# subhk/FeastKit.jl

Measured on AMD Instinct MI355X. Metric: eigenpairs/sec + max residual, 16-node contour, higher is better.
Workload: dtype f64

## Files before the change

feastkit.jl_amd/_lib.py:

```python
from __future__ import annotations

import ctypes as C
import os

_HERE = os.path.dirname(os.path.abspath(__file__))
LIB_PATH = os.environ.get("FEASTHIP_LIB") or os.path.join(_HERE, "libfeasthip.so")


class FeastHipStats(C.Structure):
    _fields_ = [
        ("seconds_total", C.c_double),
        ("seconds_solve", C.c_double),
        ("krylov_iterations", C.c_int64),
        ("spmm_calls", C.c_int64),
        ("factorizations", C.c_int64),
        ("max_rel_residual", C.c_double),
    ]

    def asdict(self):
        return {k: getattr(self, k) for k, _ in self._fields_}


class FeastHipPolicy(C.Structure):
    _fields_ = [("Emin", C.c_double), ("Emax", C.c_double), ("inner_rtol", C.c_double), ("outer_tol", C.c_double),
# ... 46 lines not shown
    "feasthip_project_dev": (_i, [_vp, _i64, _vp, _i, _i, _vp, _vp]),
    "feasthip_ritz_residual": (_i, [_vp, _i64, _vp, _vp, _vp, _i64, _i, _i, _vp, _vp]),
    "feasthip_ritz_residual_dev": (_i, [_vp, _i64, _vp, _vp, _vp, _i64, _i, _i, _vp, _vp]),
    "feasthip_matmul": (_i, [_vp, _i, _i64, _vp, _vp]),
    "feasthip_matmul_dev": (_i, [_vp, _i, _i64, _vp, _vp]),
    "feasthip_band_plan": (_i, [_vp, _vp, _vp, _vp, _vp]),
    "feasthip_direct_plan_flops": (_i, [_vp, _vp]),
    "feasthip_release_factors": (_i, [_vp]),
    "feasthip_shifted_solve": (_i, [_vp, _d, _d, _i64, _vp, _vp, _ps]),
    "feasthip_shifted_solve_dev": (_i, [_vp, _d, _d, _i64, _vp, _vp, _ps]),
    "feasthip_last_node_iterations": (_i, [_vp, _vp, _i]),
    "feasthip_last_column_iterations": (_i, [_vp, _vp, _i]),
    "feasthip_last_global_node_iterations": (_i, [_vp, _vp, _i]),
    "feasthip_last_shifted_sweep": (_i, [_vp, _vp, _vp, _vp, _vp]),
    "feasthip_last_block_sweep": (_i, [_vp, _vp, _vp, _vp, _vp]),
    "feasthip_profile_enable": (_i, [_vp, _i]),
    "feasthip_profile_reset": (_i, [_vp]),
    "feasthip_profile_get": (_i, [_vp, C.c_char_p, _pd, _pi64]),
    "feasthip_profile_set_period": (_i, [_vp, _i]),
    "feasthip_profile_get_work": (_i, [_vp, C.c_char_p, _pd]),
    "feasthip_policy_init": (_i, [_vp, _d, _d, _i, _i, _d, _d, _i, _i, _i]),
    "feasthip_policy_update": (_i, [_vp, _d, _i, _i, _vp, _i]),
    "feasthip_policy_set_aside": (_i, [_vp, _i, _vp]),
    "feasthip_policy_pick_direct_nodes": (_i, [_vp, _i, _i, _d, _d, _d, _i, _vp]),
    "feasthip_policy_filter_ratio": (_d, [_d, _d, _i, _i, _i, _d, _vp, _i]),
    "feasthip_policy_reach": (_d, [_vp, _i, _d, _d, _d]),
}

UNIQUE_ID_BYTES = 128

# ... 29 lines not shown
```

feastkit.jl_amd/csrc/fh_api.hip:

```cpp
#include "fh_common.hpp"
#include "fh_kernels.hpp"
#include "fh_dense.hpp"
#include "fh_banded.hpp"
#include "fh_eig.hpp"
#include "fh_comm.hpp"
#include "fh_cholqr.hpp"
#include "fh_knobs.hpp"
#include "../../include/feasthip.h"

#include <algorithm>
#include <chrono>
#include <thread>
#include <cmath>
#include <cstring>

int fh_get_buf(feasthip_ctx* h, const char* name, size_t bytes, void** out) {
    auto it = h->bufs.find(name);
    if (it != h->bufs.end() && it->second.second >= bytes) {
        *out = it->second.first;
        return 0;
    }
    if (it != h->bufs.end()) {
        hipStreamSynchronize(h->stream);
        hipFree(it->second.first);
// ... 434 lines not shown


struct fh_op_call {
    const void* X = nullptr; size_t x_stride = 0;
    void* Y = nullptr; size_t y_stride = 0;
    const cplx* coefA = nullptr; const cplx* coefB = nullptr;
    const void* Bvec = nullptr; size_t b_stride = 0;
    const void* U = nullptr; size_t u_stride = 0;
    int dot_mode = 0; cplx* partial1 = nullptr; cplx* partial2 = nullptr;
    const int* node_active = nullptr;
    int nodes = 1;
    int m = FH_MAX_LD;
    int uniform_coef = 0;
    int prec = 64;
    const cplx* colscale = nullptr;
};

static bool fh_row_kernel_ok(feasthip_ctx* h, int ld) {
    return h->kind == 2 && ld == 64 && !h->csr.is_complex && h->csr.rp8 && fh_knob::spmm_row();
}

static int fh_apply_operator(feasthip_ctx* h, int ld, const fh_op_call& c) {
    if (h->kind == 2) {
        fh_spmm_args a;
        a.rowptr = h->csr.rowptr; a.col = h->csr.col; a.aval = h->csr.aval; a.bval = h->csr.bval;
        a.N = (int)h->csr.N; a.nodes = c.nodes;
        a.X = c.X; a.x_node_stride = c.x_stride; a.Y = c.Y; a.y_node_stride = c.y_stride;
        a.coefA = c.coefA; a.coefB = c.coefB; a.Bvec = c.Bvec; a.b_node_stride = c.b_stride;
        a.U = c.U; a.u_node_stride = c.u_stride; a.dot_mode = c.dot_mode;
        a.partial1 = c.partial1; a.partial2 = c.partial2; a.node_active = c.node_active;
        a.counters = h->profiling ? h->d_counters : nullptr; a.m = c.m; a.uniform_coef = c.uniform_coef; a.prec = c.prec;
        const bool lds_kernel = h->csr.lcol && c.prec == 64 && fh_knob::lds_spmm() && c.nodes <= 64 && c.dot_mode != 6;
        a.nblk_rows = h->csr.nblk; a.blk_start = h->csr.blk_start; a.ext_ptr = h->csr.ext_ptr; a.ext_idx = h->csr.ext_idx;
        a.lcol = lds_kernel ? h->csr.lcol : nullptr;
        a.use_row_kernel = (fh_row_kernel_ok(h, ld) && !lds_kernel) ? 1 : 0;
        a.colscale = c.colscale;
        if (c.colscale && (lds_kernel || c.prec != 64 || h->csr.is_complex)) { h->last_error = "internal: column-scaled operand needs a gather kernel over a real matrix on complex128 panels"; return -1; }
        a.rp8 = h->csr.rp8; a.col8 = h->csr.col8; a.a8 = h->csr.a8; a.b8 = h->csr.b8;
        fh_prof_begin(h, "spmm");
        fh_launch_spmm(a, ld, h->csr.is_complex != 0, h->csr.b_identity != 0, fh_spmm_grid(a.N, ld), h->stream);
        fh_prof_end(h);
        if (a.use_row_kernel) return fh_spmm_row_grid(a.N);
        if (lds_kernel) return (8 / (ld / 16)) * fh_spmm_lds_slots(a.nblk_rows, ld);
        return fh_spmm_partials(a.N, ld);
    }
    fh_dense_op_args a;
    a.A = h->dense.A; a.B = h->dense.B; a.N = (int)h->dense.N; a.is_complex = h->dense.is_complex;
    a.nodes = c.nodes; a.X = (const cplx*)c.X; a.x_node_stride = c.x_stride; a.Y = (cplx*)c.Y; a.y_node_stride = c.y_stride;
    a.coefA = c.coefA; a.coefB = c.coefB; a.Bvec = (const cplx*)c.Bvec; a.b_node_stride = c.b_stride;
    a.U = (const cplx*)c.U; a.u_node_stride = c.u_stride; a.dot_mode = c.dot_mode;
    a.partial1 = c.partial1; a.partial2 = c.partial2; a.node_active = c.node_active;
    int nblk = fh_dense_op_nblk(a.N);
    fh_prof_begin(h, "dense_op");
    fh_launch_dense_op(a, ld, nblk, h->stream);
    fh_prof_end(h);
    return nblk;
}

static int fh_op_nblk(feasthip_ctx* h, int ld) {
    if (h->kind == 2) return std::max(std::max(fh_spmm_partials((int)h->csr.N, ld), ld == 64 ? fh_spmm_row_grid((int)h->csr.N) : 0),
                                      h->csr.lcol ? (8 / (ld / 16)) * fh_spmm_lds_slots(h->csr.nblk, ld) : 0);
    return fh_dense_op_nblk((int)h->dense.N);
}
static const int* fh_perm(feasthip_ctx* h) { return h->kind == 2 ? h->csr.perm : nullptr; }
static int64_t fh_N(feasthip_ctx* h) { return h->kind == 2 ? h->csr.N : h->dense.N; }
static bool fh_b_identity(feasthip_ctx* h) { return h->kind == 2 ? h->csr.b_identity != 0 : h->dense.b_identity != 0; }

static int fh_check_problem(feasthip_ctx* h, int64_t m, int wide = 0) {
    if (!h) return FEASTHIP_ERROR_INTERNAL;
    if (h->poisoned) { h->last_error = "handle poisoned by an earlier device failure: destroy it"; return FEASTHIP_ERROR_INTERNAL; }
    if (h->kind == 0) { h->last_error = "no matrix set (feasthip_set_dense / feasthip_set_csr)"; return FEASTHIP_ERROR_N; }
    if (m <= 0 || (!wide && m > FH_MAX_LD) || m > fh_N(h)) {
        h->last_error = wide ? "block width m must satisfy 1 <= m <= N" : "block width m must satisfy 1 <= m <= min(N, 64)";
        return FEASTHIP_ERROR_M0;
    }
// ... 182 lines not shown
}

struct fh_krylov_opts {
    cplx* sum_acc = nullptr;
    const std::vector<cplx>* wnode = nullptr;
    const cplx *shared_src = nullptr, *dznode = nullptr;
    const double *shared_lambda = nullptr, *shared_lambda_host = nullptr;
};

namespace {
struct fh_krylov_work {
    feasthip_ctx* h;
    fh_solve_result& res;
    int method, prec, ld, m, nodes, N;
    size_t panel;
    bool fused = false, lazy = false;
    void *R, *Rh, *P, *V, *S, *T, *D = nullptr, *RHS32 = nullptr, *Xk = nullptr;
    fh_krylov_scalars s;
    double *r0_64, *inv_r0;
    cplx *part1, *part2, *sp[2] = {nullptr, nullptr};
    int nblk_vec, fv_rows = 0, fv1_rows = 0;
    cplx *sum_acc = nullptr, *dfs = nullptr;
    const cplx* lazy_src = nullptr;
    fh_op_call oc;
    fh_fin_args fa;
    fh_vec_args va;
    fh_fused_fin_args ff;
    int alloc(const std::vector<cplx>& z, const std::vector<cplx>* wnode);
    int start(const std::vector<cplx>& z, const cplx* RHS, cplx* X, const fh_krylov_opts& opt);
    void bicgstab_step(), cocg_step(), cocg_fused_step(int it);
};
// ... 73 lines not shown
        fh_launch_narrow_scaled((const cplx*)R64, panel, (cplxf*)RHS32, panel, r0_64, N, ld, nblk_vec, nodes, h->stream);
        FH_CHECK(hipMemsetAsync(D, 0, (size_t)nodes * panel * sizeof(cplxf), h->stream));
        FH_CHECK(hipMemcpyAsync(R, RHS32, (size_t)nodes * panel * sizeof(cplxf), hipMemcpyDeviceToDevice, h->stream));
        Xk = D;
        std::vector<double> hr0(nl), hinv(nl);
        FH_CHECK(hipMemcpyAsync(hr0.data(), r0_64, nl * sizeof(double), hipMemcpyDeviceToHost, h->stream));
        FH_CHECK(hipStreamSynchronize(h->stream));
        for (size_t i = 0; i < nl; ++i) hinv[i] = hr0[i] > 0 ? 1.0 / hr0[i] : 0.0;
        FH_CHECK(hipMemcpyAsync(inv_r0, hinv.data(), nl * sizeof(double), hipMemcpyHostToDevice, h->stream));
        FH_CHECK(hipStreamSynchronize(h->stream));
        fa.atol_scale = inv_r0;
    }
    va.X = Xk;
    lazy = shared_start && fused && h->kind == 2 && !h->csr.is_complex && !fh_knob::no_lazy_start() &&
           (!opt.shared_lambda || opt.shared_lambda_host) && !fh_knob::lds_spmm();
    if (lazy) {
        if ((rc = fh_upload_coefs(h, "kry_fscale", fh_start_factors(z, nodes, m, ld, opt.shared_lambda_host), &dfs))) return rc;
        lazy_src = opt.shared_src;
        fh_vec_args vs = va;
        vs.Q = opt.shared_src; vs.first_scale = dfs;
        fh_launch_cocg_init_lazy(vs, ld, nblk_vec, nodes, h->stream);
    } else if (shared_start) {
        fh_vec_args vs = va;
        vs.Q = opt.shared_src; vs.lambda = opt.shared_lambda; vs.znode = opt.dznode;
        fh_launch_cocg_init_shared(vs, ld, nblk_vec, nodes, h->stream);
    } else if (method == 1 || prec == 32) {
        fh_launch_cocg_init(va, ld, nblk_vec, nodes, h->stream);
    }
    if (method == 1 || prec == 32) fa.nblk = nblk_vec;
    fh_launch_fin_init(fa, ld, nodes, h->stream);
// ... 20 lines not shown
void fh_krylov_work::cocg_step() {
    oc.X = P; oc.Y = V; oc.U = nullptr; oc.dot_mode = 4; oc.node_active = s.node_active;
    fa.nblk = fh_apply_operator(h, ld, oc);
    fh_prof_begin(h, "dot_finalize"); fh_launch_fin_alpha(fa, ld, nodes, h->stream); fh_prof_end(h);
    fh_prof_begin(h, "cocg_xr"); fh_launch_cocg_update(va, ld, nblk_vec, nodes, h->stream); fh_prof_end(h);
    fa.nblk = nblk_vec;
    fh_prof_begin(h, "dot_finalize"); fh_launch_fin_rho(fa, ld, nodes, h->stream); fh_prof_end(h);
    fh_prof_begin(h, "cocg_p");
    if (sum_acc) fh_launch_cocg_p_sum(va, ld, nodes, h->stream);
    else fh_launch_cocg_p(va, ld, nblk_vec, nodes, h->stream);
    fh_prof_end(h);
    res.op_calls += 1;
}

void fh_krylov_work::cocg_fused_step(int it) {
    const bool first_lazy = lazy && it == 0;
    oc.X = first_lazy ? (const void*)lazy_src : P; oc.x_stride = first_lazy ? 0 : panel; oc.colscale = first_lazy ? dfs : nullptr;
    oc.Y = V; oc.U = nullptr; oc.dot_mode = 6; oc.node_active = s.node_active;
    oc.partial1 = sp[0]; oc.partial2 = sp[1];
    va.first_src = first_lazy ? lazy_src : nullptr; va.first_scale = first_lazy ? dfs : nullptr;
    ff.sig = sp[0]; ff.kap = sp[1]; ff.final_check = 0;
    ff.predict_stop = (h->rtol >= 1e-3 && h->atol == 0.0) ? 1 : 0;
    ff.nblk_op = fh_apply_operator(h, ld, oc);
    ff.nblk_vec = it == 0 ? fa.nblk : ((lazy && it == 1) ? fv1_rows : fv_rows);
    fh_prof_begin(h, "dot_finalize"); fh_launch_fused_fin(ff, ld, nodes, h->stream); fh_prof_end(h);
    fh_prof_begin(h, "cocg_vec"); fh_launch_fused_vec(va, ld, h->stream); fh_prof_end(h);
    res.op_calls += 1;
}

}

static int fh_krylov(feasthip_ctx* h, int method, int prec, int ld, int m, int nodes, const std::vector<cplx>& z,
                     const cplx* RHS, cplx* X, size_t stride, fh_solve_result& res, const fh_krylov_opts& opt) {
    if (h->kind != 2) prec = 64;
    fh_krylov_work k{h, res};
// ... 736 lines not shown
        if (dzAq) FH_CHECK(hipMemcpy(dzAq, aq_all.data(), aq_all.size() * sizeof(cplx), hipMemcpyHostToDevice));
        if (dzSq) FH_CHECK(hipMemcpy(dzSq, sq_all.data(), sq_all.size() * sizeof(cplx), hipMemcpyHostToDevice));
    }
    return 0;
}

struct fh_resident_sweep {
    const cplx* Q; const cplx* eigres; cplx* P; int ld;
};

static int fh_contour_apply_impl(feasthip_ctx* h, int64_t m64, const cplx* dQ, const double* ritz_lambda,
                                 cplx* dQproj, cplx* dzAq, cplx* dzSq, int* node_status, feasthip_stats* stats,
                                 const fh_resident_sweep* rs = nullptr) {
    h->shift_panels = h->shift_used = h->shift_seed_iters = 0; h->shift_seed = -1;
    h->block_panels = h->block_used = h->block_steps_max = h->block_breakdowns = h->block_passes = 0;
    const int nr = fh_comm_nranks(h);
    int64_t c0 = 0, c1 = m64;
    if (h->col_block_hi >= 0) { c0 = std::min(h->col_block_lo, m64); c1 = std::min(std::max(h->col_block_hi, c0), m64); }
    const bool full = (c0 == 0 && c1 == m64);
    if (nr == 1 && full) {
        if (rs) {
            fh_panel_io io; io.Qp = rs->Q; io.eigres = rs->eigres; io.out = rs->P;
            return fh_contour_apply_panel(h, m64, nullptr, ritz_lambda, nullptr, nullptr, nullptr, node_status, stats, nullptr, &io);
        }
        return fh_contour_apply_local(h, m64, dQ, ritz_lambda, dQproj, dzAq, dzSq, node_status, stats);
    }
    int rc = fh_check_problem(h, m64, rs ? 0 : 1);
    if (rc) return rc;
    if (!full && (dzAq || dzSq)) { h->last_error = "contour_apply: moment matrices need the full column block"; return FEASTHIP_ERROR_M0; }
    const int N = (int)fh_N(h), m = (int)m64, nodes = h->node_count, ne = (int)h->zne.size();
// ... 1370 lines not shown
    if (seed_iterations) *seed_iterations = u ? h->shift_seed_iters : 0;
    if (spmm_node_passes) *spmm_node_passes = u ? h->shift_seed_iters : 0;
    return 0;
}

extern "C" int feasthip_last_block_sweep(feasthip_handle h, int* used, int* node_steps_max, int* breakdown_nodes, int* spmm_node_passes) {
    if (!h) return FEASTHIP_ERROR_INTERNAL;
    const bool u = h->block_panels > 0 && h->block_used == h->block_panels;
    if (used) *used = u ? 1 : 0;
    if (node_steps_max) *node_steps_max = u ? h->block_steps_max : 0;
    if (breakdown_nodes) *breakdown_nodes = u ? h->block_breakdowns : 0;
    if (spmm_node_passes) *spmm_node_passes = u ? h->block_passes : 0;
    return 0;
}

extern "C" int feasthip_last_column_iterations(feasthip_handle h, int* out, int n) {
    if (!h || !out) return FEASTHIP_ERROR_INTERNAL;
    for (int e = 0; e < n; ++e) out[e] = e < (int)h->last_col_iters.size() ? h->last_col_iters[e] : 0;
    return 0;
}

extern "C" int feasthip_profile_enable(feasthip_handle h, int enable) {
    if (!h) return FEASTHIP_ERROR_INTERNAL;
    h->profiling = enable ? 1 : 0;
    if (enable) { h->prof_host_s = 0.0; h->prof_t0 = fh_now_s(); }
    return 0;
}
extern "C" int feasthip_profile_reset(feasthip_handle h) {
    if (!h) return FEASTHIP_ERROR_INTERNAL;
    fh_prof_collect(h);
// ... 41 lines not shown
```

feastkit.jl_amd/csrc/fh_common.hpp:

```cpp
#pragma once
#include <hip/hip_runtime.h>
#include <stdint.h>
#include <string>
#include <vector>
#include <map>

struct __attribute__((aligned(16))) cplx { double x, y; };

__host__ __device__ inline cplx cmake(double a, double b) { cplx r; r.x = a; r.y = b; return r; }
__host__ __device__ inline cplx cadd(cplx a, cplx b) { return cmake(a.x + b.x, a.y + b.y); }
__host__ __device__ inline cplx csub(cplx a, cplx b) { return cmake(a.x - b.x, a.y - b.y); }
__host__ __device__ inline cplx cmul(cplx a, cplx b) { return cmake(a.x * b.x - a.y * b.y, a.x * b.y + a.y * b.x); }
__host__ __device__ inline cplx cmulc(cplx a, cplx b) {  return cmake(a.x * b.x + a.y * b.y, a.x * b.y - a.y * b.x); }
__host__ __device__ inline cplx cscale(cplx a, double s) { return cmake(a.x * s, a.y * s); }
__host__ __device__ inline cplx cconj(cplx a) { return cmake(a.x, -a.y); }
__host__ __device__ inline double cabs2(cplx a) { return a.x * a.x + a.y * a.y; }
__host__ __device__ inline cplx cdiv(cplx a, cplx b) {
    double d = b.x * b.x + b.y * b.y;
    return cmake((a.x * b.x + a.y * b.y) / d, (a.y * b.x - a.x * b.y) / d);
}
__host__ __device__ inline void cfma(cplx& acc, cplx a, cplx b) {
    acc.x += a.x * b.x - a.y * b.y;
    acc.y += a.x * b.y + a.y * b.x;
}
// ... 95 lines not shown
    fh_csr csr;
    fh_dense dense;

    std::vector<cplx> zne, wne;
    double weight_scale = 2.0;
    int real_projection = 0;
    int node_first = 0, node_count = 0;
    std::vector<int> node_ids;
    std::vector<int> node_kinds;

    int solver = 1;
    int shifted = 0;
    int shift_panels = 0, shift_used = 0, shift_seed = -1, shift_seed_iters = 0;
    int block = 0;
    int block_panels = 0, block_used = 0, block_steps_max = 0, block_breakdowns = 0, block_passes = 0;
    double rtol = 1e-12, atol = 0.0;
    int maxit = 500, restart = 30, factor_precision = 64, cache_factors = 1;

    std::vector<int> last_col_iters;
    int last_col_m = 0;
    std::vector<int> last_node_iters;
    std::vector<int> global_node_iters;

    std::map<std::string, std::pair<void*, size_t>> bufs;

    char* pin = nullptr; size_t pin_cap = 0, pin_off = 0;

    int rs_m = 0, rs_ld = 0;
    cplx* rs_P = nullptr;
    cplx* rs_basis = nullptr;
// ... 65 lines not shown
```

feastkit.jl_amd/csrc/fh_kernels.hpp:

```cpp
#pragma once
#include "fh_common.hpp"

struct fh_spmm_args {
    const int* rowptr; const int* col; const void* aval; const void* bval;
    int N; int nodes;
    const void* X; size_t x_node_stride;
    void* Y; size_t y_node_stride;
    const cplx* coefA; const cplx* coefB;
    const void* Bvec; size_t b_node_stride;
    const void* U; size_t u_node_stride;
    int dot_mode;
    cplx* partial1; cplx* partial2;
    const int* node_active;
    unsigned long long* counters;
    int m;
    int uniform_coef;
    int prec;
    const int* rp8 = nullptr; const int* col8 = nullptr; const double* a8 = nullptr; const double* b8 = nullptr;
    int use_row_kernel = 0;
    const cplx* colscale = nullptr;
    int nblk_rows; const int* blk_start; const int* ext_ptr; const int* ext_idx; const unsigned short* lcol;
};
int fh_spmm_grid(int N, int ld);
int fh_spmm_partials(int N, int ld);
int fh_spmm_row_grid(int N);
int fh_spmm_lds_slots(int nblk_rows, int ld);
void fh_launch_spmm(const fh_spmm_args& a, int ld, bool is_complex, bool bident, int nblk, hipStream_t st);

struct fh_vec_args {
    int N;
    size_t node_stride;
    void *X, *R, *Rhat, *P, *V, *S, *T;
    const cplx* Q;
    const double* lambda;
    const cplx* znode;
    fh_krylov_scalars s;
    cplx* partial1; cplx* partial2;
    int prec;
    unsigned long long* counters;
    const cplx* first_src;
    const cplx* first_scale;
    cplx* sum_acc;
    const cplx* wnode;
    const double* sum_scale;
    int nodes;
};
struct fh_fin_args {
    fh_krylov_scalars s;
    const cplx* partial1; const cplx* partial2;
    int nblk; int m;
    double rtol, atol;
    const double* atol_scale;
    int mode;
    const int* col_mask;
};
void fh_launch_init_guess(const fh_vec_args& a, int ld, int nblk, int nodes, hipStream_t st);
// ... 155 lines not shown
```

feastkit.jl_amd/csrc/fh_sparse.hip:

```cpp
#include "fh_common.hpp"
#include "fh_kernels.hpp"

#define FH_BLOCK 256
#define FH_FIN_BLOCK 1024

template <int LD>
__device__ __forceinline__ void fh_block_reduce_cols(cplx v, cplx* red, cplx* out) {
    const int t = threadIdx.x;
    red[t] = v;
    __syncthreads();
    if (t < LD) {
        cplx s = red[t];
#pragma unroll
        for (int k = 1; k < FH_BLOCK / LD; ++k) s = cadd(s, red[t + k * LD]);
        out[t] = s;
    }
    __syncthreads();
}

static inline int fh_spmm_slots(int N, int ld) {
    const int nt = ld / 16, slices = 8 / nt;
    int rows = (N + slices - 1) / slices;
    int S = (rows + 15) / 16;
    if (S > 128) S = 128;
// ... 329 lines not shown
            }
        }
        if (a.dot_mode != 0) {
            red[wave][lane][0] = d1x; red[wave][lane][1] = d1y; red[wave][lane][2] = d2x; red[wave][lane][3] = d2y;
            __syncthreads();
            if (threadIdx.x < LD) {
                double s0 = 0.0, s1 = 0.0, s2 = 0.0, s3 = 0.0;
#pragma unroll
                for (int w = 0; w < WPB; ++w) { s0 += red[w][threadIdx.x][0]; s1 += red[w][threadIdx.x][1]; s2 += red[w][threadIdx.x][2]; s3 += red[w][threadIdx.x][3]; }
                if (a.partial1) a.partial1[pbase + threadIdx.x] = cmake(s0, s1);
                if (a.partial2) a.partial2[pbase + threadIdx.x] = cmake(s2, s3);
            }
            __syncthreads();
        }
    }
}

#define FH_LDS_SLOTS (FH_SPMM_R + FH_SPMM_EXT)
#define FH_LDS_RPG (FH_SPMM_R / 16)
#define FH_SEL8(arr, s) ((s) == 0 ? arr[0] : (s) == 1 ? arr[1] : (s) == 2 ? arr[2] : (s) == 3 ? arr[3] : (s) == 4 ? arr[4] : (s) == 5 ? arr[5] : (s) == 6 ? arr[6] : arr[7])
static_assert(FH_LDS_RPG == 8, "FH_SEL8 assumes eight rows per lane group");
template <typename VT, int LD, bool BIDENT>
__global__ __launch_bounds__(FH_BLOCK, 2) void k_spmm_lds(fh_spmm_args a) {
    typedef cplx CT;
    constexpr int NT = LD / 16;
    constexpr int SLICES = 8 / NT;
    extern __shared__ cplx lds_x[];
    __shared__ cplx red[FH_BLOCK];
    __shared__ int s_list[64];
    __shared__ int s_cnt;
// ... 236 lines not shown
int fh_spmm_row_grid(int N) {
    static int per_cu = 0;
    if (!per_cu) {
        int n = 0;
        if (hipOccupancyMaxActiveBlocksPerMultiprocessor(&n, k_spmm_row<cplx, false, true>, FH_ROW_THREADS, 0) != hipSuccess || n < 1) n = 1;
        per_cu = n > FH_ROW_BLOCKS_MAX ? FH_ROW_BLOCKS_MAX : n;
    }
    int S = fh_spmm_row_groups(N, per_cu);
    const int slice_rows = (N + 7) / 8, wpb = FH_ROW_THREADS / 64;
    const int need = (slice_rows + wpb - 1) / wpb;
    if (S > need) S = need < 1 ? 1 : need;
    return 8 * S;
}

void fh_launch_spmm(const fh_spmm_args& a, int ld, bool is_complex, bool bident, int nblk, hipStream_t st) {
    if (a.use_row_kernel) {
        dim3 grid(fh_spmm_row_grid(a.N)), block(FH_ROW_THREADS);
#define FH_ROW_LAUNCH(CT_, BI_) \
        do { if (a.uniform_coef) hipLaunchKernelGGL((k_spmm_row<CT_, BI_, true>), grid, block, 0, st, a); \
             else hipLaunchKernelGGL((k_spmm_row<CT_, BI_, false>), grid, block, 0, st, a); } while (0)
        if (a.prec == 32) { if (bident) FH_ROW_LAUNCH(cplxf, true); else FH_ROW_LAUNCH(cplxf, false); }
        else { if (bident) FH_ROW_LAUNCH(cplx, true); else FH_ROW_LAUNCH(cplx, false); }
#undef FH_ROW_LAUNCH
        return;
    }
    if (a.prec == 64 && a.lcol) {
        if (is_complex) {
            if (ld == 16) launch_spmm_lds<cplx, 16>(a, bident, st);
            else if (ld == 32) launch_spmm_lds<cplx, 32>(a, bident, st);
            else launch_spmm_lds<cplx, 64>(a, bident, st);
// ... 740 lines not shown
            a.partial1[o] = cmake(s0, s1);
            a.partial2[o] = cmake(s2, 0.0);
        }
        __syncthreads();
    }
    if (SUM && any && a.counters && blockIdx.x == 0 && blockIdx.y == 0 && t < LD) atomicAdd(a.counters + 4, 1ull);
    if (SUM && any) {
#pragma unroll
        for (int j = 0; j < EMAX; ++j) {
            const size_t e = e0 + (size_t)j * stride;
            if (j < per_thread && e < total) a.sum_acc[e] = cadd(a.sum_acc[e], acc[j]);
        }
    }
}

#define FH_SV_EMAX (FH_FV_EMAX / 2)

template <int LD>
__global__ __launch_bounds__(FH_BLOCK) void k_shift_init(fh_shift_args a) {
    const size_t total = (size_t)a.N * LD;
    const int c = threadIdx.x % LD;
    const cplx fs = a.fscale[a.seed * LD + c];
    cplx d1 = cmake(0, 0), d2 = cmake(0, 0);
    for (size_t e = (size_t)blockIdx.x * FH_BLOCK + threadIdx.x; e < total; e += (size_t)gridDim.x * FH_BLOCK) {
        const cplx v = a.src[e];
        const cplx r = cmul(v, fs);
        a.R[e] = r;
        for (int n = 0; n < a.nodes; ++n) a.P[(size_t)n * a.node_stride + e] = n == a.seed ? r : cmul(v, a.fscale[n * LD + c]);
        d1 = cadd(d1, cmul(r, r));
        d2.x += cabs2(r);
// ... 385 lines not shown
}
template <typename CT, int LD>
static void launch_fused_vec_t(const fh_vec_args& a, dim3 grid, int per_thread, hipStream_t st) {
    if (a.first_src) {
        if (a.sum_acc) hipLaunchKernelGGL((k_fused_vec<CT, LD, true, true>), grid, dim3(FH_FV_THREADS), 0, st, a, per_thread);
        else hipLaunchKernelGGL((k_fused_vec<CT, LD, false, true>), grid, dim3(FH_FV_THREADS), 0, st, a, per_thread);
        return;
    }
    if (a.sum_acc) hipLaunchKernelGGL((k_fused_vec<CT, LD, true, false>), grid, dim3(FH_FV_THREADS), 0, st, a, per_thread);
    else hipLaunchKernelGGL((k_fused_vec<CT, LD, false, false>), grid, dim3(FH_FV_THREADS), 0, st, a, per_thread);
}
void fh_launch_fused_vec(const fh_vec_args& a, int ld, hipStream_t st) {
    int nblk, nseg, per;
    fh_fused_vec_geometry(a.N, ld, a.prec == 32 || a.first_src != nullptr, &nblk, &nseg, &per);
    const dim3 grid(nblk, nseg);
    if (a.prec == 32) {
        if (ld == 16) launch_fused_vec_t<cplxf, 16>(a, grid, per, st);
        else if (ld == 32) launch_fused_vec_t<cplxf, 32>(a, grid, per, st);
        else launch_fused_vec_t<cplxf, 64>(a, grid, per, st);
    } else {
        if (ld == 16) launch_fused_vec_t<cplx, 16>(a, grid, per, st);
        else if (ld == 32) launch_fused_vec_t<cplx, 32>(a, grid, per, st);
        else launch_fused_vec_t<cplx, 64>(a, grid, per, st);
    }
}
```

feastkit.jl_amd/engine.py:

```python
from __future__ import annotations

import ctypes as C

import numpy as np

from . import _lib
from ._lib import FeastHipStats, FeastHipUnavailable
from .types import FeastHipError

SOLVER_LU, SOLVER_BICGSTAB, SOLVER_GMRES, SOLVER_COCG, SOLVER_BANDED, SOLVER_SHIFTED_COCG, SOLVER_BLOCK_COCG = 0, 1, 2, 3, 4, 5, 6
_SOLVER_CODES = {"direct": SOLVER_LU, "lu": SOLVER_LU, "bicgstab": SOLVER_BICGSTAB,
                 "iterative": SOLVER_BICGSTAB, "gmres": SOLVER_GMRES, "cocg": SOLVER_COCG,
                 "banded": SOLVER_BANDED, "shifted_cocg": SOLVER_SHIFTED_COCG, "block_cocg": SOLVER_BLOCK_COCG}
MAX_BLOCK = 64


def _np_ptr(a):
    return a.ctypes.data_as(C.c_void_p) if a is not None else None


class HipEngine:
    def __init__(self, device_index: int = 0):
        import torch
        self.torch = torch
# ... 193 lines not shown

    def set_solver(self, solver="direct", rtol=1e-12, atol=0.0, maxit=500, restart=30,
                   factor_precision=64, cache_factors=True):
        if solver not in _SOLVER_CODES:
            raise ValueError(f"Unsupported solver option '{solver}'. Use :direct, :banded, :bicgstab, :cocg, :shifted_cocg, :block_cocg, :gmres, or :iterative.")
        self._chk(self.lib.feasthip_set_solver(self.h, _SOLVER_CODES[solver], float(rtol), float(atol), int(maxit),
                                               int(restart), int(factor_precision), int(bool(cache_factors))))

    def set_node_solver(self, kinds):
        if kinds is None:
            self._chk(self.lib.feasthip_set_node_solver(self.h, 0, None))
            return
        k = np.ascontiguousarray(kinds, dtype=np.int32)
        self._chk(self.lib.feasthip_set_node_solver(self.h, len(k), _np_ptr(k)))

    def set_column_mask(self, mask):
        if mask is None:
            self._chk(self.lib.feasthip_set_column_mask(self.h, 0, None))
            return
        mk = np.ascontiguousarray(mask, dtype=np.int32)
        self._chk(self.lib.feasthip_set_column_mask(self.h, len(mk), _np_ptr(mk)))

    def empty(self, m):
        return self.torch.empty((m, self.N), dtype=self.torch.complex128, device=self.device)

    def upload(self, Q):
        Qc = np.ascontiguousarray(np.asarray(Q, dtype=np.complex128).T)
        return self.torch.from_numpy(Qc).to(self.device)

    def download(self, dQ, m=None):
# ... 13 lines not shown
        self._sync_stream()
        dP = self.empty(dQ.shape[0])
        status = np.zeros(max(1, self.ne), dtype=np.int32)
        stats = FeastHipStats()
        lam = None if ritz_lambda is None else np.ascontiguousarray(ritz_lambda, dtype=np.float64)
        dA = dS = None
        if want_moments:
            dA = self.torch.zeros((m, m), dtype=self.torch.complex128, device=self.device)
            dS = self.torch.zeros((m, m), dtype=self.torch.complex128, device=self.device)
        rc = self.lib.feasthip_contour_apply_dev(
            self.h, m, C.c_void_p(dQ.data_ptr()), _np_ptr(lam), C.c_void_p(dP.data_ptr()),
            C.c_void_p(dA.data_ptr()) if dA is not None else None,
            C.c_void_p(dS.data_ptr()) if dS is not None else None,
            _np_ptr(status), C.byref(stats))
        self._chk(rc)
        self.last_stats = stats.asdict()
        if want_moments:
            return dP, status, self.last_stats, dA.cpu().numpy().T.copy(), dS.cpu().numpy().T.copy()
        return dP, status, self.last_stats

    def random_block(self, m, seed):
        self._sync_stream()
        out = self.empty(int(m))
        self._chk(self.lib.feasthip_random_block_dev(self.h, int(m), C.c_uint64(int(seed) & (2 ** 64 - 1)),
                                                     C.c_void_p(out.data_ptr())))
        return out

    def estimate_count(self, m, seed):
        self._sync_stream()
        m = int(m)
        samples = np.zeros(2 * m, dtype=np.float64)
# ... 2 lines not shown
        self._chk(self.lib.feasthip_estimate_count(self.h, m, C.c_uint64(int(seed) & (2 ** 64 - 1)),
                                                   samples.ctypes.data_as(C.POINTER(C.c_double)), _np_ptr(status),
                                                   C.byref(stats)))
        self.last_stats = stats.asdict()
        return samples[0::2] + 1j * samples[1::2], status, self.last_stats

    resident = True

    def contour_apply_resident(self, dQ, m, ritz_lambda=None):
        self._sync_stream()
        status = np.zeros(max(1, self.ne), dtype=np.int32)
        stats = FeastHipStats()
        lam = None if ritz_lambda is None else np.ascontiguousarray(ritz_lambda, dtype=np.float64)
        self._chk(self.lib.feasthip_contour_apply_resident(self.h, int(m), C.c_void_p(dQ.data_ptr()) if dQ is not None else None,
                                                           _np_ptr(lam), _np_ptr(status), C.byref(stats)))
        self.last_stats = stats.asdict()
        return status, self.last_stats

    def rr_reduce_resident(self, m, rank_tol, hermitize=True):
        rank = C.c_int(0)
        Aq = np.zeros((m, m), dtype=np.complex128, order="F")
        Bq = np.zeros((m, m), dtype=np.complex128, order="F")
        self._chk(self.lib.feasthip_rr_reduce_resident(self.h, int(m), float(rank_tol), int(bool(hermitize)), C.byref(rank),
                                                       _np_ptr(Aq), _np_ptr(Bq)))
        r = int(rank.value)
        if r == m:
            return r, Aq, Bq
        return r, np.asfortranarray(Aq.ravel(order="F")[:r * r].reshape((r, r), order="F")), \
            np.asfortranarray(Bq.ravel(order="F")[:r * r].reshape((r, r), order="F"))

    def rr_ritz_resident(self, r, V, lam, M, normalize=True, use_B=True):
# ... 157 lines not shown
```

include/feasthip.h:

```cpp
#ifndef FEASTHIP_H
#define FEASTHIP_H

#include <stdint.h>

#ifdef __cplusplus
extern "C" {
#endif

#define FEASTHIP_VERSION_MAJOR 0
#define FEASTHIP_VERSION_MINOR 1

enum {
    FEASTHIP_SUCCESS = 0,
    FEASTHIP_ERROR_N = 1,
    FEASTHIP_ERROR_M0 = 2,
    FEASTHIP_ERROR_EMIN_EMAX = 3,
    FEASTHIP_ERROR_EMID_R = 4,
    FEASTHIP_ERROR_NO_CONVERGENCE = 5,
    FEASTHIP_ERROR_MEMORY = 6,
    FEASTHIP_ERROR_INTERNAL = 7,
    FEASTHIP_ERROR_LAPACK = 8,
    FEASTHIP_ERROR_FPM = 9
};

// ... 135 lines not shown
int  feasthip_rayleigh_ritz_dev(feasthip_handle h, int64_t r, const void* dQ, double Emin, double Emax,
                                int use_B, void* dX, double* lambda_out, int* M_out, double* res_out);

int  feasthip_matmul(feasthip_handle h, int which, int64_t m, const void* X, void* Y);
int  feasthip_matmul_dev(feasthip_handle h, int which, int64_t m, const void* dX, void* dY);

int  feasthip_shifted_solve(feasthip_handle h, double z_re, double z_im, int64_t m,
                            const void* X, void* Y, feasthip_stats* stats);
int  feasthip_shifted_solve_dev(feasthip_handle h, double z_re, double z_im, int64_t m,
                                const void* dX, void* dY, feasthip_stats* stats);

int  feasthip_last_node_iterations(feasthip_handle h, int* out, int n);
int  feasthip_last_global_node_iterations(feasthip_handle h, int* out, int n);
int  feasthip_last_shifted_sweep(feasthip_handle h, int* used, int* seed_node, int* seed_iterations, int* spmm_node_passes);
int  feasthip_last_block_sweep(feasthip_handle h, int* used, int* node_steps_max, int* breakdown_nodes, int* spmm_node_passes);
int  feasthip_last_column_iterations(feasthip_handle h, int* out, int n);
int  feasthip_profile_enable(feasthip_handle h, int enable);
int  feasthip_profile_reset(feasthip_handle h);
int  feasthip_profile_get(feasthip_handle h, const char* kernel_class, double* total_ms,
                          int64_t* launches);
int  feasthip_profile_set_period(feasthip_handle h, int period);
int  feasthip_profile_get_work(feasthip_handle h, const char* kernel_class, double* work);

#ifdef __cplusplus
}
#endif
#endif
```

Before: 302.2.

## Share first-iteration SpMM across contour nodes via A*x and B*x products

On the first COCG step with a lazy shared start, all nodes apply (z_k B - A) to the same column-scaled source. The new path computes A*x and B*x once in a row kernel and forms each node's product algebraically from per-node coefficients and scales. The fused dots are taken inside that kernel, and a new vector-update kernel rebuilds q from the stored U/V. This replaces per-node sparse products with one SpMM plus cheap per-node arithmetic, at the cost of extra U/V buffer traffic and heavy register use from 16-node unrolled accumulators. It is enabled by default through a handle flag.

```diff
diff --git a/feastkit.jl_amd/_lib.py b/feastkit.jl_amd/_lib.py
--- a/feastkit.jl_amd/_lib.py
+++ b/feastkit.jl_amd/_lib.py
@@ -84,6 +84,8 @@
     "feasthip_last_global_node_iterations": (_i, [_vp, _vp, _i]),
     "feasthip_last_shifted_sweep": (_i, [_vp, _vp, _vp, _vp, _vp]),
     "feasthip_last_block_sweep": (_i, [_vp, _vp, _vp, _vp, _vp]),
+    "feasthip_set_shared_first_product": (_i, [_vp, _i]),
+    "feasthip_last_shared_first_product": (_i, [_vp, _pi]),
     "feasthip_profile_enable": (_i, [_vp, _i]),
     "feasthip_profile_reset": (_i, [_vp]),
     "feasthip_profile_get": (_i, [_vp, C.c_char_p, _pd, _pi64]),
diff --git a/feastkit.jl_amd/csrc/fh_api.hip b/feastkit.jl_amd/csrc/fh_api.hip
--- a/feastkit.jl_amd/csrc/fh_api.hip
+++ b/feastkit.jl_amd/csrc/fh_api.hip
@@ -472,6 +472,7 @@
     int uniform_coef = 0;
     int prec = 64;
     const cplx* colscale = nullptr;
+    cplx *first_u = nullptr, *first_v = nullptr;
 };
 
 static bool fh_row_kernel_ok(feasthip_ctx* h, int ld) {
@@ -492,13 +493,14 @@
         a.nblk_rows = h->csr.nblk; a.blk_start = h->csr.blk_start; a.ext_ptr = h->csr.ext_ptr; a.ext_idx = h->csr.ext_idx;
         a.lcol = lds_kernel ? h->csr.lcol : nullptr;
         a.use_row_kernel = (fh_row_kernel_ok(h, ld) && !lds_kernel) ? 1 : 0;
-        a.colscale = c.colscale;
+        a.colscale = c.colscale; a.first_u = c.first_u; a.first_v = c.first_v;
+        if (c.first_u && !(c.colscale && a.use_row_kernel && c.dot_mode == 6 && c.prec == 64)) { h->last_error = "internal: the shared first product needs the row kernel, a column scale and the fused COCG dots"; return -1; }
         if (c.colscale && (lds_kernel || c.prec != 64 || h->csr.is_complex)) { h->last_error = "internal: column-scaled operand needs a gather kernel over a real matrix on complex128 panels"; return -1; }
         a.rp8 = h->csr.rp8; a.col8 = h->csr.col8; a.a8 = h->csr.a8; a.b8 = h->csr.b8;
         fh_prof_begin(h, "spmm");
         fh_launch_spmm(a, ld, h->csr.is_complex != 0, h->csr.b_identity != 0, fh_spmm_grid(a.N, ld), h->stream);
         fh_prof_end(h);
-        if (a.use_row_kernel) return fh_spmm_row_grid(a.N);
+        if (a.use_row_kernel) return a.first_u ? fh_spmm_row_first_grid(a.N) : fh_spmm_row_grid(a.N);
         if (lds_kernel) return (8 / (ld / 16)) * fh_spmm_lds_slots(a.nblk_rows, ld);
         return fh_spmm_partials(a.N, ld);
     }
@@ -516,7 +518,7 @@
 }
 
 static int fh_op_nblk(feasthip_ctx* h, int ld) {
-    if (h->kind == 2) return std::max(std::max(fh_spmm_partials((int)h->csr.N, ld), ld == 64 ? fh_spmm_row_grid((int)h->csr.N) : 0),
+    if (h->kind == 2) return std::max(std::max(fh_spmm_partials((int)h->csr.N, ld), ld == 64 ? std::max(fh_spmm_row_grid((int)h->csr.N), fh_spmm_row_first_grid((int)h->csr.N)) : 0),
                                       h->csr.lcol ? (8 / (ld / 16)) * fh_spmm_lds_slots(h->csr.nblk, ld) : 0);
     return fh_dense_op_nblk((int)h->dense.N);
 }
@@ -729,7 +731,7 @@
     fh_solve_result& res;
     int method, prec, ld, m, nodes, N;
     size_t panel;
-    bool fused = false, lazy = false;
+    bool fused = false, lazy = false, shared_first = false;
     void *R, *Rh, *P, *V, *S, *T, *D = nullptr, *RHS32 = nullptr, *Xk = nullptr;
     fh_krylov_scalars s;
     double *r0_64, *inv_r0;
@@ -833,6 +835,8 @@
     va.X = Xk;
     lazy = shared_start && fused && h->kind == 2 && !h->csr.is_complex && !fh_knob::no_lazy_start() &&
            (!opt.shared_lambda || opt.shared_lambda_host) && !fh_knob::lds_spmm();
+    shared_first = lazy && h->shared_first && fh_row_kernel_ok(h, ld);
+    if (fused) { h->sf_panels += 1; h->sf_used += shared_first ? 1 : 0; }
     if (lazy) {
         if ((rc = fh_upload_coefs(h, "kry_fscale", fh_start_factors(z, nodes, m, ld, opt.shared_lambda_host), &dfs))) return rc;
         lazy_src = opt.shared_src;
@@ -883,11 +887,14 @@
 }
 
 void fh_krylov_work::cocg_fused_step(int it) {
-    const bool first_lazy = lazy && it == 0;
+    const bool first_lazy = lazy && it == 0, first_shared = first_lazy && shared_first;
     oc.X = first_lazy ? (const void*)lazy_src : P; oc.x_stride = first_lazy ? 0 : panel; oc.colscale = first_lazy ? dfs : nullptr;
     oc.Y = V; oc.U = nullptr; oc.dot_mode = 6; oc.node_active = s.node_active;
     oc.partial1 = sp[0]; oc.partial2 = sp[1];
     va.first_src = first_lazy ? lazy_src : nullptr; va.first_scale = first_lazy ? dfs : nullptr;
+    oc.first_u = first_shared ? (cplx*)S : nullptr; oc.first_v = (first_shared && !fh_b_identity(h)) ? (cplx*)T : nullptr;
+    va.first_u = oc.first_u; va.first_v = first_shared ? (fh_b_identity(h) ? lazy_src : (const cplx*)T) : nullptr;
+    va.coefA = oc.coefA; va.coefB = oc.coefB;
     ff.sig = sp[0]; ff.kap = sp[1]; ff.final_check = 0;
     ff.predict_stop = (h->rtol >= 1e-3 && h->atol == 0.0) ? 1 : 0;
     ff.nblk_op = fh_apply_operator(h, ld, oc);
@@ -1654,6 +1661,7 @@
                                  const fh_resident_sweep* rs = nullptr) {
     h->shift_panels = h->shift_used = h->shift_seed_iters = 0; h->shift_seed = -1;
     h->block_panels = h->block_used = h->block_steps_max = h->block_breakdowns = h->block_passes = 0;
+    h->sf_panels = h->sf_used = 0;
     const int nr = fh_comm_nranks(h);
     int64_t c0 = 0, c1 = m64;
     if (h->col_block_hi >= 0) { c0 = std::min(h->col_block_lo, m64); c1 = std::min(std::max(h->col_block_hi, c0), m64); }
@@ -3054,6 +3062,18 @@
     return 0;
 }
 
+extern "C" int feasthip_set_shared_first_product(feasthip_handle h, int on) {
+    if (!h) return FEASTHIP_ERROR_INTERNAL;
+    h->shared_first = on ? 1 : 0;
+    return 0;
+}
+
+extern "C" int feasthip_last_shared_first_product(feasthip_handle h, int* used) {
+    if (!h) return FEASTHIP_ERROR_INTERNAL;
+    if (used) *used = (h->sf_panels > 0 && h->sf_used == h->sf_panels) ? 1 : 0;
+    return 0;
+}
+
 extern "C" int feasthip_last_column_iterations(feasthip_handle h, int* out, int n) {
     if (!h || !out) return FEASTHIP_ERROR_INTERNAL;
     for (int e = 0; e < n; ++e) out[e] = e < (int)h->last_col_iters.size() ? h->last_col_iters[e] : 0;
diff --git a/feastkit.jl_amd/csrc/fh_common.hpp b/feastkit.jl_amd/csrc/fh_common.hpp
--- a/feastkit.jl_amd/csrc/fh_common.hpp
+++ b/feastkit.jl_amd/csrc/fh_common.hpp
@@ -133,6 +133,8 @@
     int shift_panels = 0, shift_used = 0, shift_seed = -1, shift_seed_iters = 0;
     int block = 0;
     int block_panels = 0, block_used = 0, block_steps_max = 0, block_breakdowns = 0, block_passes = 0;
+    int shared_first = 1;
+    int sf_panels = 0, sf_used = 0;
     double rtol = 1e-12, atol = 0.0;
     int maxit = 500, restart = 30, factor_precision = 64, cache_factors = 1;
 
diff --git a/feastkit.jl_amd/csrc/fh_kernels.hpp b/feastkit.jl_amd/csrc/fh_kernels.hpp
--- a/feastkit.jl_amd/csrc/fh_kernels.hpp
+++ b/feastkit.jl_amd/csrc/fh_kernels.hpp
@@ -19,11 +19,13 @@
     const int* rp8 = nullptr; const int* col8 = nullptr; const double* a8 = nullptr; const double* b8 = nullptr;
     int use_row_kernel = 0;
     const cplx* colscale = nullptr;
+    cplx* first_u = nullptr; cplx* first_v = nullptr;
     int nblk_rows; const int* blk_start; const int* ext_ptr; const int* ext_idx; const unsigned short* lcol;
 };
 int fh_spmm_grid(int N, int ld);
 int fh_spmm_partials(int N, int ld);
 int fh_spmm_row_grid(int N);
+int fh_spmm_row_first_grid(int N);
 int fh_spmm_lds_slots(int nblk_rows, int ld);
 void fh_launch_spmm(const fh_spmm_args& a, int ld, bool is_complex, bool bident, int nblk, hipStream_t st);
 
@@ -40,6 +42,10 @@
     unsigned long long* counters;
     const cplx* first_src;
     const cplx* first_scale;
+    const cplx* first_u;
+    const cplx* first_v;
+    const cplx* coefA;
+    const cplx* coefB;
     cplx* sum_acc;
     const cplx* wnode;
     const double* sum_scale;
diff --git a/feastkit.jl_amd/csrc/fh_sparse.hip b/feastkit.jl_amd/csrc/fh_sparse.hip
--- a/feastkit.jl_amd/csrc/fh_sparse.hip
+++ b/feastkit.jl_amd/csrc/fh_sparse.hip
@@ -367,6 +367,143 @@
             __syncthreads();
         }
     }
+}
+
+#define FH_ROW1_THREADS 512
+#define FH_ROW1_NODES 16
+
+__device__ __forceinline__ cplx fh_first_q(cplx fs, cplx ca, cplx cb, cplx u, cplx v) {
+    return cmul(fs, cadd(cmul(cb, v), cmul(ca, u)));
+}
+
+template <bool BIDENT>
+__global__ __launch_bounds__(FH_ROW1_THREADS, 2) void k_spmm_row_first(fh_spmm_args a) {
+    constexpr int LD = 64, NCH = FH_ROW1_NODES;
+    constexpr int WPB = FH_ROW1_THREADS / 64;
+    __shared__ cplx s_fs[NCH][LD];
+    __shared__ cplx s_c[NCH][2];
+    __shared__ double red[WPB][LD][4];
+    const int lane = threadIdx.x & 63;
+    const int wave = __builtin_amdgcn_readfirstlane(threadIdx.x >> 6);
+    const int S = gridDim.x >> 3;
+    const int grp = blockIdx.x & 7, slot = blockIdx.x >> 3;
+    const int slice_rows = (a.N + 7) / 8;
+    const int row_lo = min(a.N, grp * slice_rows);
+    const int row_hi = min(a.N, row_lo + slice_rows);
+    const int band = S * WPB;
+    typedef const double __attribute__((address_space(4))) * cdptr;
+    typedef const int __attribute__((address_space(4))) * ciptr;
+    const cdptr a8 = (cdptr)a.a8;
+    const cdptr b8 = (cdptr)a.b8;
+    const ciptr rp8 = (ciptr)a.rp8;
+    const ciptr col8 = (ciptr)a.col8;
+    const int prow = blockIdx.x, nprow = gridDim.x;
+    const cplx* __restrict__ X = (const cplx*)a.X;
+    cplx* __restrict__ Uo = a.first_u;
+    cplx* __restrict__ Vo = a.first_v;
+    bool stored = false;
+
+    for (int n0 = 0; n0 < a.nodes; n0 += NCH) {
+        const int nn = min(NCH, a.nodes - n0);
+        __syncthreads();
+        for (int idx = threadIdx.x; idx < nn * LD; idx += FH_ROW1_THREADS) s_fs[idx / LD][idx % LD] = a.colscale[(size_t)n0 * LD + idx];
+        if ((int)threadIdx.x < nn) {
+            s_c[threadIdx.x][0] = a.coefA[(size_t)(n0 + threadIdx.x) * LD];
+            s_c[threadIdx.x][1] = a.coefB[(size_t)(n0 + threadIdx.x) * LD];
+        }
+        unsigned mask = 0;
+        for (int n = 0; n < nn; ++n)
+            if (!a.node_active || a.node_active[n0 + n] != 0) mask |= 1u << n;
+        mask = __builtin_amdgcn_readfirstlane(mask);
+        __syncthreads();
+        double d[NCH][4];
+#pragma unroll
+        for (int n = 0; n < NCH; ++n) { d[n][0] = 0.0; d[n][1] = 0.0; d[n][2] = 0.0; d[n][3] = 0.0; }
+        if (mask != 0) {
+            if (!stored && a.counters && blockIdx.x == 0 && threadIdx.x == 0) {
+                atomicAdd(a.counters + 0, 1ull);
+                atomicAdd(a.counters + 1, (unsigned long long)(3 * LD));
+            }
+            for (int i = row_lo + slot * WPB + wave; i < row_hi; i += band) {
+                const int c0 = rp8[i], c1 = rp8[i + 1];
+                double ux = 0.0, uy = 0.0, vx = 0.0, vy = 0.0;
+                const cplx xown = (X + (size_t)i * LD)[lane];
+                for (int ch = c0; ch < c1; ++ch) {
+                    const ciptr cc = col8 + (size_t)ch * 8;
+                    const cdptr aa = a8 + (size_t)ch * 8;
+                    cplx xs[8];
+#pragma unroll
+                    for (int q = 0; q < 8; ++q) {
+                        const int j = cc[q];
+                        if (j != i) {
+                            const cplx* __restrict__ rowp = X + (size_t)j * LD;
+                            xs[q] = rowp[lane];
+                        } else {
+                            xs[q] = xown;
+                        }
+                    }
+#pragma unroll
+                    for (int q = 0; q < 8; ++q) {
+                        const cplx x = xs[q];
+                        const double av = aa[q];
+                        ux += av * x.x; uy += av * x.y;
+                        if (!BIDENT) {
+                            const double bv = (b8 + (size_t)ch * 8)[q];
+                            vx += bv * x.x; vy += bv * x.y;
+                        }
+                    }
+                }
+                const cplx u = cmake(ux, uy);
+                cplx v = cmake(vx, vy);
+                if (BIDENT) v = xown;
+                if (!stored) {
+                    fh_st_nt((Uo + (size_t)i * LD) + lane, u);
+                    if (!BIDENT) fh_st_nt((Vo + (size_t)i * LD) + lane, v);
+                }
+                int ln = lane, l0 = 0;
+                asm volatile("" : "+v"(ln), "+v"(l0));
+#pragma unroll
+                for (int n = 0; n < NCH; ++n) {
+                    if (mask & (1u << n)) {
+                        const cplx fs = s_fs[n][ln];
+                        const cplx accd = fh_first_q(fs, s_c[n][l0], s_c[n][l0 + 1], u, v);
+                        const cplx xo = cmul(fs, xown);
+                        const cplx t1 = cmul(xo, accd), t2 = cmul(accd, accd);
+                        d[n][0] += t1.x; d[n][1] += t1.y; d[n][2] += t2.x; d[n][3] += t2.y;
+                    }
+                }
+            }
+            stored = true;
+        }
+#pragma unroll
+        for (int n = 0; n < NCH; ++n) {
+            if (n < nn) {
+                const size_t pbase = ((size_t)(n0 + n) * nprow + prow) * LD;
+                if (mask & (1u << n)) {
+                    red[wave][lane][0] = d[n][0]; red[wave][lane][1] = d[n][1]; red[wave][lane][2] = d[n][2]; red[wave][lane][3] = d[n][3];
+                    __syncthreads();
+                    if (threadIdx.x < LD) {
+                        double s0 = 0.0, s1 = 0.0, s2 = 0.0, s3 = 0.0;
+#pragma unroll
+                        for (int w = 0; w < WPB; ++w) { s0 += red[w][threadIdx.x][0]; s1 += red[w][threadIdx.x][1]; s2 += red[w][threadIdx.x][2]; s3 += red[w][threadIdx.x][3]; }
+                        a.partial1[pbase + threadIdx.x] = cmake(s0, s1);
+                        a.partial2[pbase + threadIdx.x] = cmake(s2, s3);
+                    }
+                    __syncthreads();
+                } else if (threadIdx.x < LD) {
+                    a.partial1[pbase + threadIdx.x] = cmake(0, 0);
+                    a.partial2[pbase + threadIdx.x] = cmake(0, 0);
+                }
+            }
+        }
+    }
+}
+int fh_spmm_row_first_grid(int N) {
+    const int slice_rows = (N + 7) / 8, wpb = FH_ROW1_THREADS / 64;
+    const int need = (slice_rows + wpb - 1) / wpb;
+    int S = 32;
+    if (S > need) S = need < 1 ? 1 : need;
+    return 8 * S;
 }
 
 #define FH_LDS_SLOTS (FH_SPMM_R + FH_SPMM_EXT)
@@ -633,6 +770,12 @@
 }
 
 void fh_launch_spmm(const fh_spmm_args& a, int ld, bool is_complex, bool bident, int nblk, hipStream_t st) {
+    if (a.use_row_kernel && a.first_u) {
+        dim3 grid(fh_spmm_row_first_grid(a.N)), block(FH_ROW1_THREADS);
+        if (bident) hipLaunchKernelGGL((k_spmm_row_first<true>), grid, block, 0, st, a);
+        else hipLaunchKernelGGL((k_spmm_row_first<false>), grid, block, 0, st, a);
+        return;
+    }
     if (a.use_row_kernel) {
         dim3 grid(fh_spmm_row_grid(a.N)), block(FH_ROW_THREADS);
 #define FH_ROW_LAUNCH(CT_, BI_) \
@@ -1403,6 +1546,124 @@
     }
 }
 
+#define FH_FV1_NODES 16
+__global__ __launch_bounds__(FH_FV_THREADS, 2) void k_fused_vec_first(fh_vec_args a, int per_thread) {
+    constexpr int LD = 64, NCH = FH_FV1_NODES;
+    __shared__ cplx s_al[NCH][LD], s_be[NCH][LD], s_fs[NCH][LD];
+    __shared__ cplx s_c[NCH][3];
+    __shared__ double red[FH_FV_THREADS / 64][LD][3];
+    const int t = threadIdx.x, lane = t & 63, wave = t >> 6;
+    const int c = t % LD;
+    const size_t total = (size_t)a.N * LD;
+    const size_t stride = (size_t)gridDim.x * FH_FV_THREADS;
+    const size_t e0 = (size_t)blockIdx.y * stride * per_thread + (size_t)blockIdx.x * FH_FV_THREADS + t;
+    const int prow = blockIdx.y * gridDim.x + blockIdx.x, nprow = gridDim.x * gridDim.y;
+    const cplx* __restrict__ src = a.first_src;
+    const cplx* __restrict__ Up = a.first_u;
+    const cplx* __restrict__ Vp = a.first_v;
+    cplx* __restrict__ carry = (cplx*)a.Rhat;
+    bool any = false;
+    for (int n = 0; n < a.nodes; ++n)
+        if (a.s.node_accum[n] && a.s.accum[n * LD + c] != 0) any = true;
+
+    for (int n0 = 0; n0 < a.nodes; n0 += NCH) {
+        const int nn = min(NCH, a.nodes - n0);
+        const bool first_chunk = n0 == 0, last_chunk = n0 + NCH >= a.nodes;
+        __syncthreads();
+        for (int idx = t; idx < nn * LD; idx += FH_FV_THREADS) {
+            const size_t i = (size_t)n0 * LD + idx;
+            s_al[idx / LD][idx % LD] = a.s.alpha[i]; s_be[idx / LD][idx % LD] = a.s.beta[i]; s_fs[idx / LD][idx % LD] = a.first_scale[i];
+        }
+        if (t < nn) { s_c[t][0] = a.coefA[(size_t)(n0 + t) * LD]; s_c[t][1] = a.coefB[(size_t)(n0 + t) * LD]; s_c[t][2] = a.wnode[n0 + t]; }
+        unsigned nmask = 0, stepm = 0, actm = 0;
+        for (int n = 0; n < nn; ++n) {
+            if (!a.s.node_accum[n0 + n]) continue;
+            nmask |= 1u << n;
+            const int i = (n0 + n) * LD + c;
+            if (a.s.accum[i] != 0) {
+                stepm |= 1u << n;
+                if (a.s.active[i] != 0) actm |= 1u << n;
+            }
+            if (a.counters && blockIdx.x == 0 && blockIdx.y == 0 && t == 0) {
+                atomicAdd(a.counters + 2, (unsigned long long)a.s.node_accum[n0 + n]);
+                atomicAdd(a.counters + 3, (unsigned long long)a.s.node_active[n0 + n]);
+                atomicAdd(a.counters + 5, (unsigned long long)a.s.node_active[n0 + n]);
+            }
+        }
+        nmask = __builtin_amdgcn_readfirstlane(nmask);
+        __syncthreads();
+        double dd[NCH][3];
+#pragma unroll
+        for (int n = 0; n < NCH; ++n) { dd[n][0] = 0.0; dd[n][1] = 0.0; dd[n][2] = 0.0; }
+        if (any) {
+            for (int j0 = 0; j0 < per_thread; j0 += 2) {
+                cplx sv[2], uv[2], vv[2], acc[2];
+                size_t el[2];
+                bool ok[2];
+#pragma unroll
+                for (int u = 0; u < 2; ++u) {
+                    el[u] = e0 + (size_t)(j0 + u) * stride;
+                    asm volatile("" : "+v"(el[u]));
+                    ok[u] = (j0 + u < per_thread) && el[u] < total;
+                    sv[u] = cmake(0, 0); uv[u] = cmake(0, 0); vv[u] = cmake(0, 0); acc[u] = cmake(0, 0);
+                    if (ok[u]) {
+                        if (stepm) sv[u] = src[el[u]];
+                        if (actm) { uv[u] = fh_ld_nt(Up + el[u]); vv[u] = Vp[el[u]]; }
+                        if (!first_chunk) acc[u] = carry[el[u]];
+                    }
+                }
+                int cl = c, l0 = 0;
+                asm volatile("" : "+v"(cl), "+v"(l0));
+#pragma unroll
+                for (int n = 0; n < NCH; ++n) {
+                    if (!(nmask & (1u << n))) continue;
+                    if (stepm & (1u << n)) {
+                        const cplx al = s_al[n][cl], be = s_be[n][cl], fs = s_fs[n][cl];
+                        const cplx coef = cmul(s_c[n][l0 + 2], al);
+                        const bool act = (actm & (1u << n)) != 0;
+                        cplx* __restrict__ R = (cplx*)a.R + (size_t)(n0 + n) * a.node_stride;
+                        cplx* __restrict__ P = (cplx*)a.P + (size_t)(n0 + n) * a.node_stride;
+#pragma unroll
+                        for (int u = 0; u < 2; ++u) {
+                            const cplx pv = cmul(fs, sv[u]);
+                            cfma(acc[u], coef, pv);
+                            if (act && ok[u]) {
+                                const cplx qv = fh_first_q(fs, s_c[n][l0], s_c[n][l0 + 1], uv[u], vv[u]);
+                                const cplx rn = csub(pv, cmul(al, qv));
+                                R[el[u]] = rn;
+                                P[el[u]] = cadd(rn, cmul(be, pv));
+                                dd[n][0] += rn.x * rn.x - rn.y * rn.y; dd[n][1] += 2.0 * rn.x * rn.y; dd[n][2] += cabs2(rn);
+                            }
+                        }
+                    }
+                }
+#pragma unroll
+                for (int u = 0; u < 2; ++u) {
+                    if (!ok[u]) continue;
+                    if (last_chunk) a.sum_acc[el[u]] = cadd(a.sum_acc[el[u]], acc[u]);
+                    else carry[el[u]] = acc[u];
+                }
+            }
+        }
+#pragma unroll
+        for (int n = 0; n < NCH; ++n) {
+            if (!(nmask & (1u << n))) continue;
+            red[wave][lane][0] = dd[n][0]; red[wave][lane][1] = dd[n][1]; red[wave][lane][2] = dd[n][2];
+            __syncthreads();
+            if (t < LD) {
+                double s0 = 0.0, s1 = 0.0, s2 = 0.0;
+#pragma unroll
+                for (int w = 0; w < FH_FV_THREADS / 64; ++w) { s0 += red[w][t][0]; s1 += red[w][t][1]; s2 += red[w][t][2]; }
+                const size_t o = ((size_t)(n0 + n) * nprow + prow) * LD + t;
+                a.partial1[o] = cmake(s0, s1);
+                a.partial2[o] = cmake(s2, 0.0);
+            }
+            __syncthreads();
+        }
+    }
+    if (any && a.counters && blockIdx.x == 0 && blockIdx.y == 0 && t < LD) atomicAdd(a.counters + 4, 1ull);
+}
+
 #define FH_SV_EMAX (FH_FV_EMAX / 2)
 
 template <int LD>
@@ -1818,6 +2079,10 @@
     int nblk, nseg, per;
     fh_fused_vec_geometry(a.N, ld, a.prec == 32 || a.first_src != nullptr, &nblk, &nseg, &per);
     const dim3 grid(nblk, nseg);
+    if (a.first_src && a.first_u) {
+        hipLaunchKernelGGL(k_fused_vec_first, grid, dim3(FH_FV_THREADS), 0, st, a, per);
+        return;
+    }
     if (a.prec == 32) {
         if (ld == 16) launch_fused_vec_t<cplxf, 16>(a, grid, per, st);
         else if (ld == 32) launch_fused_vec_t<cplxf, 32>(a, grid, per, st);
diff --git a/feastkit.jl_amd/engine.py b/feastkit.jl_amd/engine.py
--- a/feastkit.jl_amd/engine.py
+++ b/feastkit.jl_amd/engine.py
@@ -231,6 +231,16 @@
         k = np.ascontiguousarray(kinds, dtype=np.int32)
         self._chk(self.lib.feasthip_set_node_solver(self.h, len(k), _np_ptr(k)))
 
+    def set_shared_first_product(self, on=True):
+        self._chk(self.lib.feasthip_set_shared_first_product(self.h, int(bool(on))))
+
+    def _sweep_stats(self, stats):
+        d = stats.asdict()
+        used = C.c_int(0)
+        self._chk(self.lib.feasthip_last_shared_first_product(self.h, C.byref(used)))
+        d["shared_first_product"] = bool(used.value)
+        return d
+
     def set_column_mask(self, mask):
         if mask is None:
             self._chk(self.lib.feasthip_set_column_mask(self.h, 0, None))
@@ -274,7 +284,7 @@
             C.c_void_p(dS.data_ptr()) if dS is not None else None,
             _np_ptr(status), C.byref(stats))
         self._chk(rc)
-        self.last_stats = stats.asdict()
+        self.last_stats = self._sweep_stats(stats)
         if want_moments:
             return dP, status, self.last_stats, dA.cpu().numpy().T.copy(), dS.cpu().numpy().T.copy()
         return dP, status, self.last_stats
@@ -307,7 +317,7 @@
         lam = None if ritz_lambda is None else np.ascontiguousarray(ritz_lambda, dtype=np.float64)
         self._chk(self.lib.feasthip_contour_apply_resident(self.h, int(m), C.c_void_p(dQ.data_ptr()) if dQ is not None else None,
                                                            _np_ptr(lam), _np_ptr(status), C.byref(stats)))
-        self.last_stats = stats.asdict()
+        self.last_stats = self._sweep_stats(stats)
         return status, self.last_stats
 
     def rr_reduce_resident(self, m, rank_tol, hermitize=True):
diff --git a/include/feasthip.h b/include/feasthip.h
--- a/include/feasthip.h
+++ b/include/feasthip.h
@@ -173,6 +173,8 @@
 int  feasthip_last_global_node_iterations(feasthip_handle h, int* out, int n);
 int  feasthip_last_shifted_sweep(feasthip_handle h, int* used, int* seed_node, int* seed_iterations, int* spmm_node_passes);
 int  feasthip_last_block_sweep(feasthip_handle h, int* used, int* node_steps_max, int* breakdown_nodes, int* spmm_node_passes);
+int  feasthip_set_shared_first_product(feasthip_handle h, int on);
+int  feasthip_last_shared_first_product(feasthip_handle h, int* used);
 int  feasthip_last_column_iterations(feasthip_handle h, int* out, int n);
 int  feasthip_profile_enable(feasthip_handle h, int enable);
 int  feasthip_profile_reset(feasthip_handle h);
```

Result: faster. 311.0 (median of 6 runs) (+2.9%).
